# terraytherapeutics/COATI

Measured on AMD Instinct MI355X. Metric: molecules/sec (contrastive+AR train step), grande_closed, higher is better.
Workload: dtype bf16; 1 GPU; grande_closed d=256 L=16 nh=16 + E3GNN h=256x5, V=10322, batch 1024/GPU, seq_len 80, 16-atom point clouds, InfoNCE + AR loss, bf16 MFMA operands / fp32 accumulate + fp32 master weights, random-init weights; global_batch=1024, seq_len=80, parallelism=dp1

## Files before the change

### coati_amd/csrc/engine.cpp

```cpp
#include <stdarg.h>
#include <stdio.h>
#include <stdlib.h>
#include <string.h>

#include <algorithm>
#include <string>
#include <vector>

#include "../../include/coati_hip.h"
#include "kernels.h"

#define HIPCHK(x) do { hipError_t _h = (x); if (_h != hipSuccess) { coati_set_error("%s: %s", #x, hipGetErrorString(_h)); return COATI_EHIP; } } while (0)

static thread_local char g_err[512] = "";
void coati_set_error(const char* fmt, ...) {
  va_list ap;
  va_start(ap, fmt);
  vsnprintf(g_err, sizeof(g_err), fmt, ap);
  va_end(ap);
}
extern "C" const char* coati_last_error(void) { return g_err; }
extern "C" int coati_abi_version(void) { return COATI_ABI_VERSION; }

namespace {
// ... 1908 lines not shown
  COATI_CHECK_ARG(e->have_ws, "engine_infonce: needs the workspace of a forward / encode call");
  const size_t need = (size_t)2 * B * Bg;
  const size_t dh4_floats = (size_t)e->B * (e->T1 > e->T2 ? e->T1 : e->T2) * 4 * e->cfg.n_hidden_xformer * sizeof(bf16_t) / sizeof(float);
  COATI_CHECK_SHAPE(need <= e->nce_cap || need <= dh4_floats,
                    "engine_infonce: B=%d x Bg=%d does not fit the logits scratch (workspace was sized for Bg=%zu)", B, Bg,
                    e->nce_cap / (2 * (size_t)(e->B > 0 ? e->B : 1)));
  float* L1 = need <= e->nce_cap ? e->nce : reinterpret_cast<float*>(e->dh4);
  float* L2 = L1 + (size_t)B * Bg;
  COATI_TRY(launch_count_valid(bad_all, Bg, scal + 4, scal + 7, s));
  {
    SgemmBatch sb;
    COATI_TRY(sgemm_batch_add(sb, S_loc, E, 1, C_all, 1, E, L1, Bg, B, Bg, E, nullptr, 1.f, 0));
    COATI_TRY(sgemm_batch_add(sb, C_loc, E, 1, S_all, 1, E, L2, Bg, B, Bg, E, nullptr, 1.f, 0));
    COATI_TRY(launch_sgemm_batch(sb, s));
  }
  COATI_TRY(launch_infonce_rows2(L1, L2, Bg, B, Bg, row0, bad_all, scal + 2, scal + 3, scal + 7, gscale, s));
  {
    SgemmBatch sb;
    COATI_TRY(sgemm_batch_add(sb, L1, 1, Bg, S_loc, E, 1, dC_all, E, Bg, E, B, nullptr, 1.f, 0));
    COATI_TRY(sgemm_batch_add(sb, L2, 1, Bg, C_loc, E, 1, dS_all, E, Bg, E, B, nullptr, 1.f, 0));
    COATI_TRY(launch_sgemm_batch(sb, s));
  }
  {
    SgemmBatch sb;
    COATI_TRY(sgemm_batch_add(sb, L1, Bg, 1, C_all, E, 1, dS_all + (size_t)row0 * E, E, B, E, Bg, nullptr, 1.f, 1));
    COATI_TRY(sgemm_batch_add(sb, L2, Bg, 1, S_all, E, 1, dC_all + (size_t)row0 * E, E, B, E, Bg, nullptr, 1.f, 1));
    COATI_TRY(launch_sgemm_batch(sb, s));
  }
  return COATI_OK;
}

int coati_engine_backward(coati_engine* e, const float* dh_smiles, const float* dh_e3gnn, int stage, void* stream) {
  COATI_CHECK_ARG(e && !c2_refused(e), "engine_backward: a COATI2 engine bound without gradient and Adam buffers is inference-only (no backward)");
  COATI_CHECK_ARG(e->have_fwd && e->G, "engine_backward: no forward / gradient buffer");
  COATI_CHECK_ARG(stage >= 0 && stage <= 5, "engine_backward: bad stage");
  const bool c2 = e->enc_to_coati >= 0;
  COATI_CHECK_ARG(!c2 || dh_e3gnn == nullptr, "engine_backward: a COATI2 engine has no point encoder (dh_e3gnn must be null)");
  hipStream_t s = (hipStream_t)stream;
  const coati_config& c = e->cfg;
  const int C = c.n_hidden_xformer, H = c.n_hidden_e3nn, E = c.n_embd_common, B = e->B;
  if (stage == 0 || stage == 1) {
    const int M2 = e->p2.M;
    {
      GemmArgs a;
      memset(&a, 0, sizeof(a));
      a.A = e->p2.af; a.lda = C; a.B = e->S + e->lmhead; a.ldb = C; a.M = M2; a.N = c.n_tok; a.K = C;
      a.C = e->dlogits; a.ldc = e->Vpad; a.n_store = e->Vpad; a.lse = e->ce_lse; a.target = e->p2.packed ? e->p2.ypk : e->y_next; a.scal = e->scal;
      ProfScope ps(e, SITE_LMHEAD_DLOGITS, 2.0 * M2 * c.n_tok * C, s, (double)M2 * C * 2 + (double)c.n_tok * C * 2 + (double)M2 * e->Vpad * 2);
      COATI_TRY(gemm_rows(a, 0, EPI_CE_BWD, s));
    }
    COATI_TRY(wgrad(e, SITE_LMHEAD_WGRAD, e->dlogits, 0, e->Vpad, e->p2.af, C, M2, e->Vpad, C, e->G + e->lmhead, C, nullptr, c.n_tok, s));
    HIPCHK(hipMemsetAsync(e->dcliptok, 0, (size_t)B * E * sizeof(float), s));
    COATI_TRY(xformer_bwd(e, e->p2, e->da, 0, e->dcliptok, s, -1, 0, e->dlogits));
    if (dh_e3gnn) HIPCHK(hipMemcpyAsync(e->dhe, dh_e3gnn, (size_t)B * E * sizeof(float), hipMemcpyDeviceToDevice, s));
    else HIPCHK(hipMemsetAsync(e->dhe, 0, (size_t)B * E * sizeof(float), s));
    if (dh_smiles) HIPCHK(hipMemcpyAsync(e->dhs, dh_smiles, (size_t)B * E * sizeof(float), hipMemcpyDeviceToDevice, s));
    else HIPCHK(hipMemsetAsync(e->dhs, 0, (size_t)B * E * sizeof(float), s));
    if (c2) {
      COATI_TRY(launch_axpy(e->dcliptok, e->dhs, 1.f, (long long)B * E, s));
      COATI_TRY(coati2_head_bwd(e, e->c2t, e->c2t_sv, e->h_smiles, e->dcliptok, e->dhs, e->dhs, B, true, s));
      if (e->enc_to_coati > 0)
        COATI_TRY(coati2_head_bwd(e, e->c2s, e->c2s_sv, e->hstop, e->dhs, e->c2s.residual ? e->dhs : nullptr, e->dhstop, B, true, s));
    } else if (c.token_mlp) {
      HIPCHK(hipMemsetAsync(e->dptok, 0, (size_t)B * E * sizeof(float), s));
      HIPCHK(hipMemsetAsync(e->dstok, 0, (size_t)B * E * sizeof(float), s));
      COATI_TRY(launch_select_rows_bwd(e->use_point, e->dcliptok, e->dptok, e->dstok, B, E, s));
      SgemmBatch sb;
      COATI_TRY(head_linear_bwd(e, sb, e->dptok, e->sa, e->tokw, e->tokb, e->dsa, B, E, E));
      COATI_TRY(head_linear_bwd(e, sb, e->dstok, e->sb, e->tokw, e->tokb, e->dsb, B, E, E));
      COATI_TRY(launch_sgemm_batch(sb, s));
      COATI_TRY(launch_silu_bwd(e->h_e3gnn, e->dsa, e->dhe, (long long)B * E, 1, s));
      COATI_TRY(launch_silu_bwd(e->h_smiles, e->dsb, e->dhs, (long long)B * E, 1, s));
    } else {
      COATI_TRY(launch_select_rows_bwd(e->use_point, e->dcliptok, e->dhe, e->dhs, B, E, s));
    }
    const bool old_arch = c.norm_clips && c.old_architecture;
    if (e->enc_to_coati <= 0) {
    if (old_arch) {
      COATI_TRY(launch_layernorm_bwd(e->dhs, 1, E, e->hs_ln, E, 0, e->hs_mean, e->hs_rstd, e->P + e->s2c_lnw, nullptr, e->dhs_ln, nullptr, e->G + e->s2c_lnw, e->G + e->s2c_lnb, e->ln_partial, B, E, s));
      if (c.use_point_encoder)
        COATI_TRY(launch_layernorm_bwd(e->dhe, 1, E, e->hp_ln, E, 0, e->hp_mean, e->hp_rstd, e->P + e->p2c_lnw, nullptr, e->dhp_ln, nullptr, e->G + e->p2c_lnw, e->G + e->p2c_lnb, e->ln_partial, B, E, s));
    }
    {
      SgemmBatch sb;
      if (old_arch) COATI_TRY(head_linear_bwd(e, sb, e->dhs_ln, e->hstop, e->s2c_w, e->s2c_b, e->dhstop, B, E, C));
      else if (c.norm_clips) COATI_TRY(head_linear_bwd(e, sb, e->dhs, e->hs_ln, e->s2c_w, e->s2c_b, e->dhs_ln, B, E, C));
      else COATI_TRY(head_linear_bwd(e, sb, e->dhs, e->hstop, e->s2c_w, e->s2c_b, e->dhstop, B, E, C));
      if (c.use_point_encoder) {
        if (old_arch) COATI_TRY(head_linear_bwd(e, sb, e->dhp_ln, e->hpoint, e->p2c_w, e->p2c_b, e->dhpoint, B, E, H));
        else if (c.norm_clips) COATI_TRY(head_linear_bwd(e, sb, e->dhe, e->hp_ln, e->p2c_w, e->p2c_b, e->dhp_ln, B, E, H));
        else COATI_TRY(head_linear_bwd(e, sb, e->dhe, e->hpoint, e->p2c_w, e->p2c_b, e->dhpoint, B, E, H));
      }
      COATI_TRY(launch_sgemm_batch(sb, s));
    }
    if (c.norm_clips && !old_arch) {
      COATI_TRY(launch_layernorm_bwd(e->dhs_ln, 1, C, e->hstop, C, 0, e->hs_mean, e->hs_rstd, e->P + e->s2c_lnw, nullptr, e->dhstop, nullptr, e->G + e->s2c_lnw, e->G + e->s2c_lnb, e->ln_partial, B, C, s));
      if (c.use_point_encoder)
        COATI_TRY(launch_layernorm_bwd(e->dhp_ln, 1, H, e->hpoint, H, 0, e->hp_mean, e->hp_rstd, e->P + e->p2c_lnw, nullptr, e->dhpoint, nullptr, e->G + e->p2c_lnw, e->G + e->p2c_lnb, e->ln_partial, B, H, s));
    }
    }
  }
  const int Lx = c.n_layer_xformer, Lmid = Lx / 2;
  const bool ovl_bwd = (stage == 0 || stage == 2 || stage == 4) && (e->prof_mask == 0 || e->prof_keep_overlap) && c.use_point_encoder;
  if (stage == 0 || stage == 1) { e->gnn_bwd_done = false; e->gnn_side_pending = false; }
  if (ovl_bwd) {
    COATI_TRY(fork_side(e, s));
    COATI_TRY(gnn_bwd(e, e->dhpoint, e->side));
  }
  if (stage == 0 || stage == 2 || stage == 4) {
    if (e->p1.tail) {
      COATI_TRY(xformer_bwd(e, e->p1, e->dhstop, 1, nullptr, s, Lx, stage == 4 ? Lmid : 0));
    } else {
      float* dxf = reinterpret_cast<float*>(e->dh4);
      HIPCHK(hipMemsetAsync(dxf, 0, (size_t)e->p1.M * C * sizeof(float), s));
      COATI_TRY(launch_scatter_rows_add(e->dhstop, e->stop_pos, dxf, B, e->T1, C, s, e->p1.packed ? e->p1.off : nullptr));
      COATI_TRY(xformer_bwd(e, e->p1, dxf, 1, nullptr, s, Lx, stage == 4 ? Lmid : 0));
    }
  }
  if (stage == 5) COATI_TRY(xformer_bwd(e, e->p1, nullptr, 1, nullptr, s, Lmid, 0));
  if (ovl_bwd && stage == 4) {
    e->gnn_side_pending = true;
  } else if (ovl_bwd || (stage == 5 && e->gnn_side_pending)) {
    COATI_TRY(join_side(e, s));
    e->gnn_bwd_done = true;
    e->gnn_side_pending = false;
// ... 352 lines not shown
```

### coati_amd/csrc/gnn.hip

```cpp
#include "kernels.h"

#define IN_EPS 1e-5f

__global__ __launch_bounds__(256) void gnn_embed_kernel(const long long* __restrict__ atoms, const int* __restrict__ lut_ix,
                                                        const int* __restrict__ lut_iy, const float* __restrict__ W,
                                                        const float* __restrict__ bias, float* __restrict__ h32,
                                                        bf16_t* __restrict__ h16, long long ld16, float* __restrict__ rstd_out,
                                                        float* __restrict__ mask, int BA, int H, int* __restrict__ err) {
  const int lane = threadIdx.x & 63, wave = threadIdx.x >> 6;
  const int row = blockIdx.x * 4 + wave;
  if (row >= BA) return;
  long long z = atoms[row];
  if (lane == 0) mask[row] = z > 0 ? 1.f : 0.f;
  if (lut_ix == nullptr && z > 83 && lane == 0 && err != nullptr) atomicOr(err, 4);
  if (z < 0) z = 0;
  if (z > 119) z = 119;
  const bool table = lut_ix == nullptr;
  if (table && z > 83) z = 83;
  const int ix = table ? 0 : lut_ix[z], iy = table ? 0 : lut_iy[z];
  float e[16];
  float s = 0.f;
#pragma unroll
  for (int i = 0; i < 16; ++i) {
    const int c = lane + 64 * i;
    float v = 0.f;
    if (c < H) {
      if (table) {
        v = W[z * H + c];
      } else {
        v = bias[c];
        if (ix >= 0) v += W[c * 28 + ix];
        if (iy >= 0) v += W[c * 28 + iy];
      }
    }
    e[i] = v;
    s += v;
  }
  const float mean = wave_sum(s) / (float)H;
  float q = 0.f;
#pragma unroll
  for (int i = 0; i < 16; ++i)
    if (lane + 64 * i < H) q += (e[i] - mean) * (e[i] - mean);
  const float rstd = 1.0f / sqrtf(wave_sum(q) / (float)H + IN_EPS);
  if (lane == 0) rstd_out[row] = rstd;
#pragma unroll
  for (int i = 0; i < 16; ++i) {
    const int c = lane + 64 * i;
    if (c < H) {
      const float v = (e[i] - mean) * rstd;
      h32[(long long)row * H + c] = v;
      h16[(long long)row * ld16 + c] = f2bf(v);
    }
  }
}

int launch_gnn_embed(const long long* atoms, const int* lut_ix, const int* lut_iy, const float* W, const float* b,
                     float* h32, bf16_t* h16, long long ld16, float* rstd, float* mask, int BA, int H,
                     hipStream_t s, int* err) {
  COATI_CHECK_ARG(atoms && W && h32 && h16 && rstd && mask && ((lut_ix && lut_iy && b) || (!lut_ix && !lut_iy && !b)), "gnn_embed: null operand");
  COATI_CHECK_SHAPE(BA > 0 && H > 0 && H <= 1024, "gnn_embed: unsupported shape");
  hipLaunchKernelGGL(gnn_embed_kernel, dim3(cdiv(BA, 4)), dim3(256), 0, s, atoms, lut_ix, lut_iy, W, b, h32, h16, ld16, rstd, mask, BA, H, err);
  COATI_LAUNCH_CHECK("gnn_embed");
  return COATI_OK;
}

__global__ __launch_bounds__(256) void gnn_embed_bwd_kernel(const long long* __restrict__ atoms, const int* __restrict__ lut_ix,
                                                            const int* __restrict__ lut_iy, const float* __restrict__ de,
                                                            float* __restrict__ dW, float* __restrict__ db, int BA, int H,
                                                            int rows_per_chunk) {
  extern __shared__ float acc[];
  for (int i = threadIdx.x; i < 29 * H; i += blockDim.x) acc[i] = 0.f;
  __syncthreads();
  const int r0 = blockIdx.x * rows_per_chunk;
  int r1 = r0 + rows_per_chunk;
  if (r1 > BA) r1 = BA;
  for (int c = threadIdx.x; c < H; c += blockDim.x) {
    float bsum = 0.f;
    for (int row = r0; row < r1; ++row) {
      long long z = atoms[row];
      if (z < 0) z = 0;
      if (z > 119) z = 119;
      const int ix = lut_ix[z], iy = lut_iy[z];
      const float v = de[(long long)row * H + c];
      bsum += v;
      acc[ix * H + c] += v;
      if (iy != ix) acc[iy * H + c] += v;
    }
    acc[28 * H + c] = bsum;
  }
  __syncthreads();
  for (int f = threadIdx.x; f < 28 * H; f += blockDim.x) {
    const int c = f / 28, i = f - c * 28;
    const float v = acc[i * H + c];
    if (v != 0.f) atomicAdd(dW + f, v);
  }
  for (int c = threadIdx.x; c < H; c += blockDim.x) atomicAdd(db + c, acc[28 * H + c]);
}

__global__ __launch_bounds__(256) void gnn_embed_table_bwd_kernel(const long long* __restrict__ atoms, const float* __restrict__ de,
                                                                  float* __restrict__ dT, int BA, int H, int rows_per_chunk) {
  const int r0 = blockIdx.x * rows_per_chunk;
  int r1 = r0 + rows_per_chunk;
  if (r1 > BA) r1 = BA;
  for (int c = threadIdx.x; c < H; c += blockDim.x) {
    float run = 0.f;
    long long zr = -1;
    for (int row = r0; row < r1; ++row) {
      long long z = atoms[row];
      if (z < 0) z = 0;
      if (z > 83) z = 83;
      if (z != zr) {
        if (zr >= 0 && run != 0.f) atomicAdd(dT + zr * H + c, run);
        zr = z;
        run = 0.f;
      }
      run += de[(long long)row * H + c];
    }
    if (zr >= 0 && run != 0.f) atomicAdd(dT + zr * H + c, run);
  }
}

int launch_gnn_embed_bwd(const long long* atoms, const int* lut_ix, const int* lut_iy, const float* de,
                         float* dW, float* db, int BA, int H, hipStream_t s) {
  if (lut_ix == nullptr && lut_iy == nullptr && db == nullptr) {
    COATI_CHECK_ARG(atoms && de && dW, "gnn_embed_bwd: null operand");
    const int rpc = 32;
    hipLaunchKernelGGL(gnn_embed_table_bwd_kernel, dim3(cdiv(BA, rpc)), dim3(256), 0, s, atoms, de, dW, BA, H, rpc);
    COATI_LAUNCH_CHECK("gnn_embed_table_bwd");
    return COATI_OK;
  }
  COATI_CHECK_ARG(atoms && lut_ix && lut_iy && de && dW && db, "gnn_embed_bwd: null operand");
  COATI_CHECK_SHAPE((size_t)29 * H * 4 <= 64 * 1024, "gnn_embed_bwd: H=%d too wide for the LDS accumulator", H);
  const int chunks = BA >= 4096 ? 128 : (BA >= 256 ? 8 : 1);
  const int rpc = cdiv(BA, chunks);
  hipLaunchKernelGGL(gnn_embed_bwd_kernel, dim3(cdiv(BA, rpc)), dim3(256), (size_t)29 * H * 4, s, atoms, lut_ix, lut_iy, de, dW, db, BA, H, rpc);
  COATI_LAUNCH_CHECK("gnn_embed_bwd");
  return COATI_OK;
}

__global__ __launch_bounds__(256) void gnn_node_res_silu_kernel(const float* __restrict__ u32, const long long* __restrict__ atoms,
                                                                const int* __restrict__ lut_ix, const int* __restrict__ lut_iy,
                                                                const float* __restrict__ W3c, long long ldw, bf16_t* __restrict__ upre,
                                                                bf16_t* __restrict__ t16, int BA, int H) {
  const int row = blockIdx.x;
  if (row >= BA) return;
  long long z = atoms[row];
  if (z < 0) z = 0;
  if (z > 119) z = 119;
  const int ix = lut_ix[z], iy = lut_iy[z];
  for (int c = threadIdx.x; c < H; c += blockDim.x) {
    float v = u32[(long long)row * H + c];
    if (ix >= 0) v += W3c[c * ldw + ix];
    if (iy >= 0 && iy != ix) v += W3c[c * ldw + iy];
    upre[(long long)row * H + c] = f2bf(v);
    t16[(long long)row * H + c] = f2bf(silu_f(v));
  }
}

int launch_gnn_node_res_silu(const float* u32, const long long* atoms, const int* lut_ix, const int* lut_iy, const float* W3c, long long ldw,
                             bf16_t* upre, bf16_t* t16, int BA, int H, hipStream_t s) {
  COATI_CHECK_ARG(u32 && atoms && lut_ix && lut_iy && W3c && upre && t16, "gnn_node_res_silu: null operand");
  hipLaunchKernelGGL(gnn_node_res_silu_kernel, dim3(BA), dim3(256), 0, s, u32, atoms, lut_ix, lut_iy, W3c, ldw, upre, t16, BA, H);
  COATI_LAUNCH_CHECK("gnn_node_res_silu");
  return COATI_OK;
}

__global__ __launch_bounds__(256) void gnn_onehot_wgrad_kernel(const long long* __restrict__ atoms, const int* __restrict__ lut_ix,
                                                               const int* __restrict__ lut_iy, const bf16_t* __restrict__ du,
                                                               float* __restrict__ dW, long long ldw, int BA, int H, int rows_per_chunk) {
  extern __shared__ float acc[];
  for (int i = threadIdx.x; i < 28 * H; i += blockDim.x) acc[i] = 0.f;
// ... 385 lines not shown
```

### coati_amd/csrc/kernels.h

```cpp
#pragma once
#include "common.h"

enum CoatiEpi {
  EPI_BF16 = 0,
  EPI_F32 = 1,
  EPI_RES_F32 = 2,
  EPI_GELU = 3,
  EPI_DGELU = 4,
  EPI_SILU = 5,
  EPI_DSILU = 6,
  EPI_ACC_F32 = 7,
  EPI_CE_PARTIAL = 8,
  EPI_CE_BWD = 9,
  EPI_EDGE_DPRE = 10,
  EPI_QKV_ROPE = 11,
  EPI_GELU_GRAD = 12,
  EPI_MUL_AUX = 13,
  EPI_LNBWD = 14,
  EPI_CE_BWD_ROW = 15,
  EPI_CE_LSE = 16,
  EPI_COUNT = 17
};

struct GemmArgs {
// ... 224 lines not shown
int launch_topk_sample_prompt(const float* logits, long long ldl, int B, int V, int k, float inv_temp, const float* u,
                              const long long* prompt, long long ldp, const int* plen, int pos, long long* tok_out, int* stopped,
                              int stop_token, int pad_token, hipStream_t s);
int launch_topk_sample_rows(const float* logits, long long ldl, int B, int V, int k, float inv_temp, const float* u, long long ldu,
                            const long long* prompt, long long ldp, const int* plen, const int* req, int* pos, long long* out,
                            long long ldo, long long* tok_next, int* done, int Tmax, int stop_token, hipStream_t s);
int launch_kv_cache_fill_rows(const bf16_t* qkv, bf16_t* cache, const int* row_src, int R, int B, int T, int n_head, int head_size,
                              int Tmax, hipStream_t s);
int launch_gather_last_rows(const float* x, const int* off, float* out, int B, int C, int R, hipStream_t s);
int launch_kv_cache_fill(const bf16_t* qkv, bf16_t* cache, int B, int m, int n_head, int head_size, int Tmax, hipStream_t s);
int launch_batch_ncols(const long long* tok, int B, int S, int* ncols, hipStream_t s);
int launch_batch_tail(const long long* tok, int B, int S, int ncol, long long* tok_out, long long* y_out,
                      const long long* masked, int n_masked, hipStream_t s);

int launch_ce_finish(const float2* partial, int tiles_n, const bf16_t* a, long long lda, const bf16_t* W,
                     long long ldw, const long long* target, float* lse, float* scal, int M, int C, int V,
                     hipStream_t s);
int launch_ce_lse_finish(const bf16_t* a, long long lda, const bf16_t* W, long long ldw, const long long* target, const float* lse,
                         float* scal, int M, int C, int V, hipStream_t s);
int launch_ce_lse_finish_picked(const long long* target, const float* lse, const float* tl, float* scal, int M, int V, hipStream_t s);
int launch_ce_seq(const float2* partial, int tiles_n, const bf16_t* a, long long lda, const bf16_t* W, long long ldw,
                  const long long* target, const int* off, float* nll, int B, int T, int C, int V, hipStream_t s);
int launch_ce_seq_bwd(const float2* partial, int tiles_n, const bf16_t* a, long long lda, const bf16_t* W, long long ldw,
                      const long long* target, const int* off, const float* weights, float* nll, float* lse, float* row_scale, int B, int T,
                      int C, int V, hipStream_t s);

int launch_gnn_embed(const long long* atoms, const int* lut_ix, const int* lut_iy, const float* W, const float* b,
                     float* h32, bf16_t* h16, long long ld16, float* rstd, float* mask, int BA, int H,
                     hipStream_t s, int* err = nullptr);
int launch_gnn_node_res_silu(const float* u32, const long long* atoms, const int* lut_ix, const int* lut_iy, const float* W3c, long long ldw,
                             bf16_t* upre, bf16_t* t16, int BA, int H, hipStream_t s);
int launch_gnn_onehot_wgrad(const long long* atoms, const int* lut_ix, const int* lut_iy, const bf16_t* du, float* dW, long long ldw, int BA,
                            int H, hipStream_t s);
int launch_gnn_embed_bwd(const long long* atoms, const int* lut_ix, const int* lut_iy, const float* de,
                         float* dW, float* db, int BA, int H, hipStream_t s);
int launch_gnn_geom(const float* coords, const float* mask, float cutoff, float* d2, float* w, int B, int A,
                    hipStream_t s);
int launch_gnn_compact(const float* w_dense, const float* d2_dense, int* seg, int* n_edges, int* e_bj, int* e_bk, int* e_rev,
                       float* e_d2, float* e_w, int* pos, int B, int A, hipStream_t s);
int launch_gnn_edge_pre_c(const bf16_t* P, long long ldp, const int* seg, const int* e_bk, const float* e_d2, const float* w1c,
                          long long w1c_stride, const float* b1, bf16_t* e1, int BA, int H, hipStream_t s);
int launch_gnn_edge_reduce_c(const bf16_t* s2, const int* seg, const float* e_w, bf16_t* mi, long long ldmi, int BA, int H, hipStream_t s);
int launch_gnn_edge_fwd_fused(const bf16_t* P, long long ldp, const int* seg, const int* e_bk, const float* e_d2, const float* e_w,
                              const float* w1c, long long w1c_stride, const float* b1, const bf16_t* W3, long long ldw, const float* b3,
                              bf16_t* e1, bf16_t* s2, bf16_t* mi, long long ldmi, int BA, int H, hipStream_t s);
int launch_gnn_edge_reduce_bwd_c(const bf16_t* dmi, long long lddmi, const bf16_t* s2, const int* seg, const float* e_w,
                                 bf16_t* ds2, int BA, int H, hipStream_t s);
int launch_gnn_edge_pre_bwd_c(const bf16_t* dpre, const int* seg, const int* e_rev, const float* e_d2, bf16_t* dP, long long lddp,
                              float* dw1c, long long dw1c_stride, float* db1, int BA, int H, hipStream_t s);
int launch_gnn_readout(const float* o, const float* mask, float* hp, int B, int A, int H, hipStream_t s);
int launch_gnn_readout_bwd(const float* dhp, const float* mask, bf16_t* dout, int B, int A, int H, hipStream_t s);

int launch_silu_fwd(const float* x, float* y, long long n, hipStream_t s);
int launch_silu_bwd(const float* x, const float* dy, float* dx, long long n, int accumulate, hipStream_t s);
int launch_swiglu(const float* u, long long ldu, float* g, long long ldg, int B, int N, hipStream_t s);
int launch_swiglu_bwd(const float* u, long long ldu, const float* dg, long long lddg, float* du, long long lddu, int B, int N, hipStream_t s);
int launch_group_mean_rows(const float* x, long long ldx, const int* off, const float* w, const float* fallback, float* out, int G, int E,
                           hipStream_t s);
int launch_select_rows(const unsigned char* use_a, const float* a, const float* b, float* out, int B, int C,
                       hipStream_t s);
int launch_select_rows_bwd(const unsigned char* use_a, const float* dout, float* da, float* db, int B, int C,
                           hipStream_t s);
int launch_axpy(const float* x, float* y, float alpha, long long n, hipStream_t s);
int launch_infonce_rows2(float* logits, float* logits2, long long ld, int R, int N, int label0, const unsigned char* bad,
                         float* loss_sum, float* loss_sum2, const float* inv_count, float gscale, hipStream_t s);
int launch_infonce_rows(float* logits, long long ld, int R, int N, int label0, const unsigned char* bad,
                        float* loss_sum, const float* inv_count, float gscale, hipStream_t s);
int launch_count_valid(const unsigned char* bad, int n, float* out_count, float* out_inv, hipStream_t s);
int launch_colsum2(const float* a, const float* b2, const unsigned char* bad, float* out, int B, int E, hipStream_t s);
int launch_center_rows(const float* z, const unsigned char* bad, const float* sum, const float* count, float* zc, int B, int E, hipStream_t s);
int launch_standardize(const float* z, const unsigned char* bad, const float* stats, const float* count, float* zt, float* rsigma,
                       int B, int E, hipStream_t s);
int launch_barlow_dc(float* C, const float* count, float lam, float* loss, int E, hipStream_t s);
int launch_standardize_bwd(const float* dzt, const float* zt, const unsigned char* bad, const float* rsigma, const float* m,
                           const float* count, float scale, float* dz, int B, int E, hipStream_t s);

int launch_grad_sqnorm(const float* g, long long n, float* partial, int n_partial, float* out_norm, float max_norm,
                       float* out_coef, hipStream_t s);
int launch_adamw(float* p, const float* g, float* m, float* v, bf16_t* shadow, long long n, float lr, float b1,
                 float b2, float eps, float wd, int step, const float* coef, float gscale, hipStream_t s, const int* skip = nullptr);
int launch_cast_bf16(const float* src, bf16_t* dst, long long n, hipStream_t s);
int launch_transpose_cast(const float* src, long long ld_src, bf16_t* dst, long long ld_dst, int rows, int cols,
                          hipStream_t s);
int launch_pack_rows_cast(const float* src, long long ld_src, bf16_t* dst, long long ld_dst, int rows, int cols,
                          hipStream_t s);

struct ShadowJob {
  long long src_off, dst_off;
  int ld_src, ld_dst, rows, cols, transpose;
};
int launch_shadow_jobs(const ShadowJob* jobs, const int* tile_start, int n_jobs, int n_tiles, const float* P, bf16_t* S,
                       hipStream_t s);
```

### coati_amd/csrc/loss.hip

```cpp
#include "kernels.h"

__global__ void silu_fwd_kernel(const float* __restrict__ x, float* __restrict__ y, long long n) {
  const long long i = (long long)blockIdx.x * blockDim.x + threadIdx.x;
  if (i < n) y[i] = silu_f(x[i]);
}
int launch_silu_fwd(const float* x, float* y, long long n, hipStream_t s) {
  COATI_CHECK_ARG(x && y, "silu_fwd: null operand");
  hipLaunchKernelGGL(silu_fwd_kernel, dim3(cdiv(n, 256)), dim3(256), 0, s, x, y, n);
  COATI_LAUNCH_CHECK("silu_fwd");
  return COATI_OK;
}

template <bool V4>
__global__ __launch_bounds__(256) void swiglu_kernel(const float* __restrict__ u, long long ldu, float* __restrict__ g, long long ldg,
                                                     int B, int N) {
  const int W = V4 ? N / 4 : N;
  const long long i = (long long)blockIdx.x * blockDim.x + threadIdx.x;
  if (i >= (long long)B * W) return;
  const long long b = i / W;
  const int j = (int)(i - b * W);
  const float* r = u + b * ldu;
  if constexpr (V4) {
    const float4 x = *reinterpret_cast<const float4*>(r + 4 * j);
    const float4 q = *reinterpret_cast<const float4*>(r + N + 4 * j);
// ... 35 lines not shown
    float4 dx, dq;
    swiglu_bwd_f(x.x, q.x, d.x, dx.x, dq.x);
    swiglu_bwd_f(x.y, q.y, d.y, dx.y, dq.y);
    swiglu_bwd_f(x.z, q.z, d.z, dx.z, dq.z);
    swiglu_bwd_f(x.w, q.w, d.w, dx.w, dq.w);
    *reinterpret_cast<float4*>(o + 4 * j) = dx;
    *reinterpret_cast<float4*>(o + N + 4 * j) = dq;
  } else {
    swiglu_bwd_f(r[j], r[N + j], dg[b * lddg + j], o[j], o[N + j]);
  }
}
int launch_swiglu_bwd(const float* u, long long ldu, const float* dg, long long lddg, float* du, long long lddu, int B, int N, hipStream_t s) {
  COATI_CHECK_ARG(u && dg && du, "swiglu_bwd: null operand");
  COATI_CHECK_SHAPE(B > 0 && N > 0 && ldu >= 2LL * N && lddg >= N && lddu >= 2LL * N, "swiglu_bwd: bad shape B=%d N=%d ldu=%lld lddg=%lld lddu=%lld", B, N,
                    ldu, lddg, lddu);
  const bool v4 = N % 4 == 0 && ldu % 4 == 0 && lddg % 4 == 0 && lddu % 4 == 0 && reinterpret_cast<uintptr_t>(u) % 16 == 0 &&
                  reinterpret_cast<uintptr_t>(dg) % 16 == 0 && reinterpret_cast<uintptr_t>(du) % 16 == 0;
  const long long n = (long long)B * (v4 ? N / 4 : N);
  if (v4) hipLaunchKernelGGL(swiglu_bwd_kernel<true>, dim3(cdiv(n, 256)), dim3(256), 0, s, u, ldu, dg, lddg, du, lddu, B, N);
  else hipLaunchKernelGGL(swiglu_bwd_kernel<false>, dim3(cdiv(n, 256)), dim3(256), 0, s, u, ldu, dg, lddg, du, lddu, B, N);
  COATI_LAUNCH_CHECK("swiglu_bwd");
  return COATI_OK;
}

__global__ __launch_bounds__(256) void group_mean_rows_kernel(const float* __restrict__ x, long long ldx, const int* __restrict__ off,
                                                              const float* __restrict__ w, const float* __restrict__ fallback,
                                                              float* __restrict__ out, int E) {
  const int g = blockIdx.x;
  const int lo = off[g], hi = off[g + 1];
  float* o = out + (long long)g * E;
  if (hi <= lo) {
    for (int e = threadIdx.x; e < E; e += blockDim.x) o[e] = fallback[(long long)g * E + e];
    return;
  }
  float ws = 0.f;
  for (int i = lo; i < hi; ++i) ws += w ? w[i] : 1.f;
  const float inv = 1.f / ws;
  for (int e = threadIdx.x; e < E; e += blockDim.x) {
    float acc = 0.f;
    for (int i = lo; i < hi; ++i) acc += (w ? w[i] : 1.f) * x[(long long)i * ldx + e];
    o[e] = acc * inv;
  }
}
int launch_group_mean_rows(const float* x, long long ldx, const int* off, const float* w, const float* fallback, float* out, int G, int E,
                           hipStream_t s) {
  COATI_CHECK_ARG(x && off && fallback && out, "group_mean_rows: null operand");
  COATI_CHECK_SHAPE(G > 0 && E > 0 && ldx >= E, "group_mean_rows: bad shape G=%d E=%d ldx=%lld", G, E, ldx);
  hipLaunchKernelGGL(group_mean_rows_kernel, dim3(G), dim3(E < 256 ? (E + 63) / 64 * 64 : 256), 0, s, x, ldx, off, w, fallback, out, E);
  COATI_LAUNCH_CHECK("group_mean_rows");
  return COATI_OK;
}

__global__ void silu_bwd_kernel(const float* __restrict__ x, const float* __restrict__ dy, float* __restrict__ dx,
                                long long n, int accumulate) {
  const long long i = (long long)blockIdx.x * blockDim.x + threadIdx.x;
  if (i < n) {
    const float g = dy[i] * dsilu_f(x[i]);
    dx[i] = accumulate ? dx[i] + g : g;
  }
}
int launch_silu_bwd(const float* x, const float* dy, float* dx, long long n, int accumulate, hipStream_t s) {
  COATI_CHECK_ARG(x && dy && dx, "silu_bwd: null operand");
  hipLaunchKernelGGL(silu_bwd_kernel, dim3(cdiv(n, 256)), dim3(256), 0, s, x, dy, dx, n, accumulate);
  COATI_LAUNCH_CHECK("silu_bwd");
  return COATI_OK;
}

__global__ void select_rows_kernel(const unsigned char* __restrict__ use_a, const float* __restrict__ a,
                                   const float* __restrict__ b, float* __restrict__ out, int B, int C) {
  const long long i = (long long)blockIdx.x * blockDim.x + threadIdx.x;
  if (i < (long long)B * C) out[i] = use_a[i / C] ? a[i] : b[i];
}
int launch_select_rows(const unsigned char* use_a, const float* a, const float* b, float* out, int B, int C, hipStream_t s) {
  COATI_CHECK_ARG(use_a && a && b && out, "select_rows: null operand");
  hipLaunchKernelGGL(select_rows_kernel, dim3(cdiv((long long)B * C, 256)), dim3(256), 0, s, use_a, a, b, out, B, C);
  COATI_LAUNCH_CHECK("select_rows");
  return COATI_OK;
}

__global__ void select_rows_bwd_kernel(const unsigned char* __restrict__ use_a, const float* __restrict__ dout,
                                       float* __restrict__ da, float* __restrict__ db, int B, int C) {
  const long long i = (long long)blockIdx.x * blockDim.x + threadIdx.x;
  if (i < (long long)B * C) {
    if (use_a[i / C]) da[i] += dout[i]; else db[i] += dout[i];
  }
}
int launch_select_rows_bwd(const unsigned char* use_a, const float* dout, float* da, float* db, int B, int C, hipStream_t s) {
  COATI_CHECK_ARG(use_a && dout && da && db, "select_rows_bwd: null operand");
  hipLaunchKernelGGL(select_rows_bwd_kernel, dim3(cdiv((long long)B * C, 256)), dim3(256), 0, s, use_a, dout, da, db, B, C);
  COATI_LAUNCH_CHECK("select_rows_bwd");
  return COATI_OK;
}

__global__ void axpy_kernel(const float* __restrict__ x, float* __restrict__ y, float alpha, long long n) {
  const long long i = (long long)blockIdx.x * blockDim.x + threadIdx.x;
  if (i < n) y[i] += alpha * x[i];
}
int launch_axpy(const float* x, float* y, float alpha, long long n, hipStream_t s) {
  COATI_CHECK_ARG(x && y, "axpy: null operand");
  hipLaunchKernelGGL(axpy_kernel, dim3(cdiv(n, 256)), dim3(256), 0, s, x, y, alpha, n);
  COATI_LAUNCH_CHECK("axpy");
  return COATI_OK;
}

template <int NR>
__global__ __launch_bounds__(256) void infonce_rows_kernel(float* __restrict__ logits, float* __restrict__ logits2, long long ld, int R, int N,
                                                           int label0, const unsigned char* __restrict__ bad, float* __restrict__ loss_sum,
                                                           float* __restrict__ loss_sum2, const float* __restrict__ inv_count, float gscale) {
  const int lane = threadIdx.x & 63, r = blockIdx.x * 4 + (threadIdx.x >> 6);
  if (r >= R) return;
  float* row = (blockIdx.y ? logits2 : logits) + (long long)r * ld;
  float* ls = blockIdx.y ? loss_sum2 : loss_sum;
  const int label = label0 + r;
  if (bad[label]) {
    for (int c = lane; c < N; c += 64) row[c] = 0.f;
    return;
  }
  const float g = gscale * inv_count[0];
  if constexpr (NR > 0) {
    float v[NR];
#pragma unroll
    for (int i = 0; i < NR; ++i) v[i] = lane + 64 * i < N ? row[lane + 64 * i] : -INFINITY;
    float mx = -INFINITY;
#pragma unroll
    for (int i = 0; i < NR; ++i) mx = fmaxf(mx, v[i]);
    mx = wave_max(mx);
    float sm = 0.f;
#pragma unroll
    for (int i = 0; i < NR; ++i) sm += __expf(v[i] - mx);
    sm = wave_sum(sm);
    const float lse = mx + __logf(sm);
    float at_label = 0.f;
#pragma unroll
    for (int i = 0; i < NR; ++i) {
      const int c = lane + 64 * i;
      float p = __expf(v[i] - lse);
      if (c == label) { at_label = v[i]; p -= 1.f; }
      if (c < N) row[c] = p * g;
    }
    at_label = wave_sum(at_label);
    if (lane == 0) atomicAdd(ls, lse - at_label);
  } else {
    float mx = -INFINITY;
    for (int c = lane; c < N; c += 64) mx = fmaxf(mx, row[c]);
    mx = wave_max(mx);
    float sm = 0.f;
    for (int c = lane; c < N; c += 64) sm += __expf(row[c] - mx);
    sm = wave_sum(sm);
    const float lse = mx + __logf(sm);
    if (lane == 0) atomicAdd(ls, lse - row[label]);
    __builtin_amdgcn_wave_barrier();
    for (int c = lane; c < N; c += 64) {
      float p = __expf(row[c] - lse);
      if (c == label) p -= 1.f;
      row[c] = p * g;
    }
  }
}
int launch_infonce_rows2(float* logits, float* logits2, long long ld, int R, int N, int label0, const unsigned char* bad,
                         float* loss_sum, float* loss_sum2, const float* inv_count, float gscale, hipStream_t s) {
  COATI_CHECK_ARG(logits && bad && loss_sum && inv_count && (logits2 == nullptr || loss_sum2 != nullptr), "infonce_rows: null operand");
  COATI_CHECK_SHAPE(R > 0 && N > 0 && label0 >= 0 && label0 + R <= N, "infonce_rows: labels out of range");
  const dim3 grid(cdiv(R, 4), logits2 ? 2 : 1);
  if (N <= 64 * 16) hipLaunchKernelGGL(infonce_rows_kernel<16>, grid, dim3(256), 0, s, logits, logits2, ld, R, N, label0, bad, loss_sum, loss_sum2, inv_count, gscale);
  else if (N <= 64 * 32) hipLaunchKernelGGL(infonce_rows_kernel<32>, grid, dim3(256), 0, s, logits, logits2, ld, R, N, label0, bad, loss_sum, loss_sum2, inv_count, gscale);
  else hipLaunchKernelGGL(infonce_rows_kernel<0>, grid, dim3(256), 0, s, logits, logits2, ld, R, N, label0, bad, loss_sum, loss_sum2, inv_count, gscale);
  COATI_LAUNCH_CHECK("infonce_rows");
  return COATI_OK;
}
int launch_infonce_rows(float* logits, long long ld, int R, int N, int label0, const unsigned char* bad,
                        float* loss_sum, const float* inv_count, float gscale, hipStream_t s) {
  return launch_infonce_rows2(logits, nullptr, ld, R, N, label0, bad, loss_sum, nullptr, inv_count, gscale, s);
}

__global__ void count_valid_kernel(const unsigned char* __restrict__ bad, int n, float* __restrict__ out_count,
                                   float* __restrict__ out_inv) {
  __shared__ int red[4];
  int c = 0;
  for (int i = threadIdx.x; i < n; i += blockDim.x) c += bad[i] ? 0 : 1;
  for (int o = 32; o > 0; o >>= 1) c += __shfl_xor(c, o, 64);
  if ((threadIdx.x & 63) == 0) red[threadIdx.x >> 6] = c;
  __syncthreads();
  if (threadIdx.x == 0) {
    const int t = red[0] + red[1] + red[2] + red[3];
    out_count[0] = (float)t;
    out_inv[0] = t > 0 ? 1.0f / (float)t : 0.f;
  }
}
int launch_count_valid(const unsigned char* bad, int n, float* out_count, float* out_inv, hipStream_t s) {
  COATI_CHECK_ARG(bad && out_count && out_inv, "count_valid: null operand");
  hipLaunchKernelGGL(count_valid_kernel, dim3(1), dim3(256), 0, s, bad, n, out_count, out_inv);
  COATI_LAUNCH_CHECK("count_valid");
  return COATI_OK;
}

__global__ __launch_bounds__(256) void colsum2_kernel(const float* __restrict__ a, const float* __restrict__ b2,
                                                      const unsigned char* __restrict__ bad, float* __restrict__ out, int B, int E) {
  __shared__ float red[2][4][64];
  const int c = blockIdx.x * 64 + (threadIdx.x & 63), rg = threadIdx.x >> 6;
  float s1 = 0.f, s2 = 0.f;
  if (c < E)
    for (int r = rg; r < B; r += 4) {
      if (bad[r]) continue;
      const float x = a[(long long)r * E + c];
      s1 += x;
      s2 += x * (b2 ? b2[(long long)r * E + c] : x);
    }
  red[0][rg][threadIdx.x & 63] = s1;
  red[1][rg][threadIdx.x & 63] = s2;
  __syncthreads();
  if (rg == 0 && c < E) {
    const int t = threadIdx.x;
    out[c] = red[0][0][t] + red[0][1][t] + red[0][2][t] + red[0][3][t];
    out[E + c] = red[1][0][t] + red[1][1][t] + red[1][2][t] + red[1][3][t];
  }
}
int launch_colsum2(const float* a, const float* b2, const unsigned char* bad, float* out, int B, int E, hipStream_t s) {
  COATI_CHECK_ARG(a && bad && out, "colsum2: null operand");
  hipLaunchKernelGGL(colsum2_kernel, dim3(cdiv(E, 64)), dim3(256), 0, s, a, b2, bad, out, B, E);
// ... 80 lines not shown
```

Baseline: 49870 molecules/s.

## Fuse grad-buffer init into select/silu bwd, batch atom loads, block-reduce InfoNCE loss

Several small backward-pass changes land together. The token_mlp head path drops four memset/memcpy calls: select_rows_bwd now writes fresh values, and silu_bwd writes base+grad directly. The GNN embedding backward kernels load atom indices once per 64-row tile, broadcast them with readlane, and batch eight gradient loads per step to cut serial dependent loads. InfoNCE moves to 8-wave blocks and reduces the loss in shared memory, so it issues one atomic per block instead of one per row.

```diff
diff --git a/coati_amd/csrc/engine.cpp b/coati_amd/csrc/engine.cpp
--- a/coati_amd/csrc/engine.cpp
+++ b/coati_amd/csrc/engine.cpp
@@ -1984,25 +1984,26 @@
     COATI_TRY(wgrad(e, SITE_LMHEAD_WGRAD, e->dlogits, 0, e->Vpad, e->p2.af, C, M2, e->Vpad, C, e->G + e->lmhead, C, nullptr, c.n_tok, s));
     HIPCHK(hipMemsetAsync(e->dcliptok, 0, (size_t)B * E * sizeof(float), s));
     COATI_TRY(xformer_bwd(e, e->p2, e->da, 0, e->dcliptok, s, -1, 0, e->dlogits));
-    if (dh_e3gnn) HIPCHK(hipMemcpyAsync(e->dhe, dh_e3gnn, (size_t)B * E * sizeof(float), hipMemcpyDeviceToDevice, s));
-    else HIPCHK(hipMemsetAsync(e->dhe, 0, (size_t)B * E * sizeof(float), s));
-    if (dh_smiles) HIPCHK(hipMemcpyAsync(e->dhs, dh_smiles, (size_t)B * E * sizeof(float), hipMemcpyDeviceToDevice, s));
-    else HIPCHK(hipMemsetAsync(e->dhs, 0, (size_t)B * E * sizeof(float), s));
+    const bool dh_fresh = !c2 && c.token_mlp;
+    if (!dh_fresh) {
+      if (dh_e3gnn) HIPCHK(hipMemcpyAsync(e->dhe, dh_e3gnn, (size_t)B * E * sizeof(float), hipMemcpyDeviceToDevice, s));
+      else HIPCHK(hipMemsetAsync(e->dhe, 0, (size_t)B * E * sizeof(float), s));
+      if (dh_smiles) HIPCHK(hipMemcpyAsync(e->dhs, dh_smiles, (size_t)B * E * sizeof(float), hipMemcpyDeviceToDevice, s));
+      else HIPCHK(hipMemsetAsync(e->dhs, 0, (size_t)B * E * sizeof(float), s));
+    }
     if (c2) {
       COATI_TRY(launch_axpy(e->dcliptok, e->dhs, 1.f, (long long)B * E, s));
       COATI_TRY(coati2_head_bwd(e, e->c2t, e->c2t_sv, e->h_smiles, e->dcliptok, e->dhs, e->dhs, B, true, s));
       if (e->enc_to_coati > 0)
         COATI_TRY(coati2_head_bwd(e, e->c2s, e->c2s_sv, e->hstop, e->dhs, e->c2s.residual ? e->dhs : nullptr, e->dhstop, B, true, s));
     } else if (c.token_mlp) {
-      HIPCHK(hipMemsetAsync(e->dptok, 0, (size_t)B * E * sizeof(float), s));
-      HIPCHK(hipMemsetAsync(e->dstok, 0, (size_t)B * E * sizeof(float), s));
-      COATI_TRY(launch_select_rows_bwd(e->use_point, e->dcliptok, e->dptok, e->dstok, B, E, s));
+      COATI_TRY(launch_select_rows_bwd(e->use_point, e->dcliptok, e->dptok, e->dstok, B, E, s, 1));
       SgemmBatch sb;
       COATI_TRY(head_linear_bwd(e, sb, e->dptok, e->sa, e->tokw, e->tokb, e->dsa, B, E, E));
       COATI_TRY(head_linear_bwd(e, sb, e->dstok, e->sb, e->tokw, e->tokb, e->dsb, B, E, E));
       COATI_TRY(launch_sgemm_batch(sb, s));
-      COATI_TRY(launch_silu_bwd(e->h_e3gnn, e->dsa, e->dhe, (long long)B * E, 1, s));
-      COATI_TRY(launch_silu_bwd(e->h_smiles, e->dsb, e->dhs, (long long)B * E, 1, s));
+      COATI_TRY(launch_silu_bwd(e->h_e3gnn, e->dsa, e->dhe, (long long)B * E, 2, s, dh_e3gnn));
+      COATI_TRY(launch_silu_bwd(e->h_smiles, e->dsb, e->dhs, (long long)B * E, 2, s, dh_smiles));
     } else {
       COATI_TRY(launch_select_rows_bwd(e->use_point, e->dcliptok, e->dhe, e->dhs, B, E, s));
     }
diff --git a/coati_amd/csrc/gnn.hip b/coati_amd/csrc/gnn.hip
--- a/coati_amd/csrc/gnn.hip
+++ b/coati_amd/csrc/gnn.hip
@@ -64,6 +64,7 @@
   return COATI_OK;
 }
 
+#define GNN_EB_DEPTH 8
 __global__ __launch_bounds__(256) void gnn_embed_bwd_kernel(const long long* __restrict__ atoms, const int* __restrict__ lut_ix,
                                                             const int* __restrict__ lut_iy, const float* __restrict__ de,
                                                             float* __restrict__ dW, float* __restrict__ db, int BA, int H,
@@ -71,22 +72,41 @@
   extern __shared__ float acc[];
   for (int i = threadIdx.x; i < 29 * H; i += blockDim.x) acc[i] = 0.f;
   __syncthreads();
+  const int lane = threadIdx.x & 63;
   const int r0 = blockIdx.x * rows_per_chunk;
   int r1 = r0 + rows_per_chunk;
   if (r1 > BA) r1 = BA;
-  for (int c = threadIdx.x; c < H; c += blockDim.x) {
+  for (int cb = 0; cb < H; cb += blockDim.x) {
+    const int c = cb + threadIdx.x;
+    const bool on = c < H;
     float bsum = 0.f;
-    for (int row = r0; row < r1; ++row) {
-      long long z = atoms[row];
-      if (z < 0) z = 0;
-      if (z > 119) z = 119;
-      const int ix = lut_ix[z], iy = lut_iy[z];
-      const float v = de[(long long)row * H + c];
-      bsum += v;
-      acc[ix * H + c] += v;
-      if (iy != ix) acc[iy * H + c] += v;
-    }
-    acc[28 * H + c] = bsum;
+    for (int rt = r0; rt < r1; rt += 64) {
+      int my_ix = -1, my_iy = -1;
+      if (rt + lane < r1) {
+        long long z = atoms[rt + lane];
+        if (z < 0) z = 0;
+        if (z > 119) z = 119;
+        my_ix = lut_ix[z];
+        my_iy = lut_iy[z];
+      }
+      const int n = r1 - rt < 64 ? r1 - rt : 64;
+      for (int j0 = 0; j0 < n; j0 += GNN_EB_DEPTH) {
+        float v[GNN_EB_DEPTH];
+#pragma unroll
+        for (int u = 0; u < GNN_EB_DEPTH; ++u) v[u] = (on && j0 + u < n) ? de[(long long)(rt + j0 + u) * H + c] : 0.f;
+#pragma unroll
+        for (int u = 0; u < GNN_EB_DEPTH; ++u) {
+          if (j0 + u >= n) break;
+          const int ix = __builtin_amdgcn_readlane(my_ix, j0 + u), iy = __builtin_amdgcn_readlane(my_iy, j0 + u);
+          if (on) {
+            bsum += v[u];
+            if (ix >= 0) acc[ix * H + c] += v[u];
+            if (iy >= 0 && iy != ix) acc[iy * H + c] += v[u];
+          }
+        }
+      }
+    }
+    if (on) acc[28 * H + c] = bsum;
   }
   __syncthreads();
   for (int f = threadIdx.x; f < 28 * H; f += blockDim.x) {
@@ -99,24 +119,42 @@
 
 __global__ __launch_bounds__(256) void gnn_embed_table_bwd_kernel(const long long* __restrict__ atoms, const float* __restrict__ de,
                                                                   float* __restrict__ dT, int BA, int H, int rows_per_chunk) {
+  const int lane = threadIdx.x & 63;
   const int r0 = blockIdx.x * rows_per_chunk;
   int r1 = r0 + rows_per_chunk;
   if (r1 > BA) r1 = BA;
-  for (int c = threadIdx.x; c < H; c += blockDim.x) {
+  for (int cb = 0; cb < H; cb += blockDim.x) {
+    const int c = cb + threadIdx.x;
+    const bool on = c < H;
     float run = 0.f;
-    long long zr = -1;
-    for (int row = r0; row < r1; ++row) {
-      long long z = atoms[row];
-      if (z < 0) z = 0;
-      if (z > 83) z = 83;
-      if (z != zr) {
-        if (zr >= 0 && run != 0.f) atomicAdd(dT + zr * H + c, run);
-        zr = z;
-        run = 0.f;
-      }
-      run += de[(long long)row * H + c];
-    }
-    if (zr >= 0 && run != 0.f) atomicAdd(dT + zr * H + c, run);
+    int zr = -1;
+    for (int rt = r0; rt < r1; rt += 64) {
+      int my_z = 0;
+      if (rt + lane < r1) {
+        long long z = atoms[rt + lane];
+        if (z < 0) z = 0;
+        if (z > 83) z = 83;
+        my_z = (int)z;
+      }
+      const int n = r1 - rt < 64 ? r1 - rt : 64;
+      for (int j0 = 0; j0 < n; j0 += GNN_EB_DEPTH) {
+        float v[GNN_EB_DEPTH];
+#pragma unroll
+        for (int u = 0; u < GNN_EB_DEPTH; ++u) v[u] = (on && j0 + u < n) ? de[(long long)(rt + j0 + u) * H + c] : 0.f;
+#pragma unroll
+        for (int u = 0; u < GNN_EB_DEPTH; ++u) {
+          if (j0 + u >= n) break;
+          const int z = __builtin_amdgcn_readlane(my_z, j0 + u);
+          if (z != zr) {
+            if (on && zr >= 0 && run != 0.f) atomicAdd(dT + (long long)zr * H + c, run);
+            zr = z;
+            run = 0.f;
+          }
+          run += v[u];
+        }
+      }
+    }
+    if (on && zr >= 0 && run != 0.f) atomicAdd(dT + (long long)zr * H + c, run);
   }
 }
 
diff --git a/coati_amd/csrc/kernels.h b/coati_amd/csrc/kernels.h
--- a/coati_amd/csrc/kernels.h
+++ b/coati_amd/csrc/kernels.h
@@ -300,7 +300,7 @@
 int launch_gnn_readout_bwd(const float* dhp, const float* mask, bf16_t* dout, int B, int A, int H, hipStream_t s);
 
 int launch_silu_fwd(const float* x, float* y, long long n, hipStream_t s);
-int launch_silu_bwd(const float* x, const float* dy, float* dx, long long n, int accumulate, hipStream_t s);
+int launch_silu_bwd(const float* x, const float* dy, float* dx, long long n, int accumulate, hipStream_t s, const float* base = nullptr);
 int launch_swiglu(const float* u, long long ldu, float* g, long long ldg, int B, int N, hipStream_t s);
 int launch_swiglu_bwd(const float* u, long long ldu, const float* dg, long long lddg, float* du, long long lddu, int B, int N, hipStream_t s);
 int launch_group_mean_rows(const float* x, long long ldx, const int* off, const float* w, const float* fallback, float* out, int G, int E,
@@ -308,7 +308,7 @@
 int launch_select_rows(const unsigned char* use_a, const float* a, const float* b, float* out, int B, int C,
                        hipStream_t s);
 int launch_select_rows_bwd(const unsigned char* use_a, const float* dout, float* da, float* db, int B, int C,
-                           hipStream_t s);
+                           hipStream_t s, int fresh = 0);
 int launch_axpy(const float* x, float* y, float alpha, long long n, hipStream_t s);
 int launch_infonce_rows2(float* logits, float* logits2, long long ld, int R, int N, int label0, const unsigned char* bad,
                          float* loss_sum, float* loss_sum2, const float* inv_count, float gscale, hipStream_t s);
diff --git a/coati_amd/csrc/loss.hip b/coati_amd/csrc/loss.hip
--- a/coati_amd/csrc/loss.hip
+++ b/coati_amd/csrc/loss.hip
@@ -111,16 +111,17 @@
 }
 
 __global__ void silu_bwd_kernel(const float* __restrict__ x, const float* __restrict__ dy, float* __restrict__ dx,
-                                long long n, int accumulate) {
+                                long long n, int accumulate, const float* __restrict__ base) {
   const long long i = (long long)blockIdx.x * blockDim.x + threadIdx.x;
   if (i < n) {
     const float g = dy[i] * dsilu_f(x[i]);
-    dx[i] = accumulate ? dx[i] + g : g;
-  }
-}
-int launch_silu_bwd(const float* x, const float* dy, float* dx, long long n, int accumulate, hipStream_t s) {
-  COATI_CHECK_ARG(x && dy && dx, "silu_bwd: null operand");
-  hipLaunchKernelGGL(silu_bwd_kernel, dim3(cdiv(n, 256)), dim3(256), 0, s, x, dy, dx, n, accumulate);
+    if (accumulate == 2) dx[i] = (base ? base[i] : 0.f) + g;
+    else dx[i] = accumulate ? dx[i] + g : g;
+  }
+}
+int launch_silu_bwd(const float* x, const float* dy, float* dx, long long n, int accumulate, hipStream_t s, const float* base) {
+  COATI_CHECK_ARG(x && dy && dx && accumulate >= 0 && accumulate <= 2 && (accumulate == 2 || !base), "silu_bwd: null operand / bad mode");
+  hipLaunchKernelGGL(silu_bwd_kernel, dim3(cdiv(n, 256)), dim3(256), 0, s, x, dy, dx, n, accumulate, base);
   COATI_LAUNCH_CHECK("silu_bwd");
   return COATI_OK;
 }
@@ -138,15 +139,24 @@
 }
 
 __global__ void select_rows_bwd_kernel(const unsigned char* __restrict__ use_a, const float* __restrict__ dout,
-                                       float* __restrict__ da, float* __restrict__ db, int B, int C) {
+                                       float* __restrict__ da, float* __restrict__ db, int B, int C, int fresh) {
   const long long i = (long long)blockIdx.x * blockDim.x + threadIdx.x;
   if (i < (long long)B * C) {
-    if (use_a[i / C]) da[i] += dout[i]; else db[i] += dout[i];
-  }
-}
-int launch_select_rows_bwd(const unsigned char* use_a, const float* dout, float* da, float* db, int B, int C, hipStream_t s) {
+    const bool a = use_a[i / C] != 0;
+    if (fresh) {
+      const float v = 0.f + dout[i];
+      da[i] = a ? v : 0.f;
+      db[i] = a ? 0.f : v;
+    } else if (a) {
+      da[i] += dout[i];
+    } else {
+      db[i] += dout[i];
+    }
+  }
+}
+int launch_select_rows_bwd(const unsigned char* use_a, const float* dout, float* da, float* db, int B, int C, hipStream_t s, int fresh) {
   COATI_CHECK_ARG(use_a && dout && da && db, "select_rows_bwd: null operand");
-  hipLaunchKernelGGL(select_rows_bwd_kernel, dim3(cdiv((long long)B * C, 256)), dim3(256), 0, s, use_a, dout, da, db, B, C);
+  hipLaunchKernelGGL(select_rows_bwd_kernel, dim3(cdiv((long long)B * C, 256)), dim3(256), 0, s, use_a, dout, da, db, B, C, fresh);
   COATI_LAUNCH_CHECK("select_rows_bwd");
   return COATI_OK;
 }
@@ -162,68 +172,79 @@
   return COATI_OK;
 }
 
+#define NCE_WAVES 8
 template <int NR>
-__global__ __launch_bounds__(256) void infonce_rows_kernel(float* __restrict__ logits, float* __restrict__ logits2, long long ld, int R, int N,
+__global__ __launch_bounds__(64 * NCE_WAVES) void infonce_rows_kernel(float* __restrict__ logits, float* __restrict__ logits2, long long ld, int R, int N,
                                                            int label0, const unsigned char* __restrict__ bad, float* __restrict__ loss_sum,
                                                            float* __restrict__ loss_sum2, const float* __restrict__ inv_count, float gscale) {
-  const int lane = threadIdx.x & 63, r = blockIdx.x * 4 + (threadIdx.x >> 6);
-  if (r >= R) return;
-  float* row = (blockIdx.y ? logits2 : logits) + (long long)r * ld;
-  float* ls = blockIdx.y ? loss_sum2 : loss_sum;
-  const int label = label0 + r;
-  if (bad[label]) {
-    for (int c = lane; c < N; c += 64) row[c] = 0.f;
-    return;
-  }
-  const float g = gscale * inv_count[0];
-  if constexpr (NR > 0) {
-    float v[NR];
-#pragma unroll
-    for (int i = 0; i < NR; ++i) v[i] = lane + 64 * i < N ? row[lane + 64 * i] : -INFINITY;
-    float mx = -INFINITY;
-#pragma unroll
-    for (int i = 0; i < NR; ++i) mx = fmaxf(mx, v[i]);
-    mx = wave_max(mx);
-    float sm = 0.f;
-#pragma unroll
-    for (int i = 0; i < NR; ++i) sm += __expf(v[i] - mx);
-    sm = wave_sum(sm);
-    const float lse = mx + __logf(sm);
-    float at_label = 0.f;
-#pragma unroll
-    for (int i = 0; i < NR; ++i) {
-      const int c = lane + 64 * i;
-      float p = __expf(v[i] - lse);
-      if (c == label) { at_label = v[i]; p -= 1.f; }
-      if (c < N) row[c] = p * g;
+  __shared__ float red[NCE_WAVES];
+  const int lane = threadIdx.x & 63, wave = threadIdx.x >> 6, r = blockIdx.x * NCE_WAVES + wave;
+  float term = 0.f;
+  if (r < R) {
+    float* row = (blockIdx.y ? logits2 : logits) + (long long)r * ld;
+    const int label = label0 + r;
+    if (bad[label]) {
+      for (int c = lane; c < N; c += 64) row[c] = 0.f;
+    } else {
+      const float g = gscale * inv_count[0];
+      if constexpr (NR > 0) {
+        float v[NR];
+#pragma unroll
+        for (int i = 0; i < NR; ++i) v[i] = lane + 64 * i < N ? row[lane + 64 * i] : -INFINITY;
+        float mx = -INFINITY;
+#pragma unroll
+        for (int i = 0; i < NR; ++i) mx = fmaxf(mx, v[i]);
+        mx = wave_max(mx);
+        float sm = 0.f;
+#pragma unroll
+        for (int i = 0; i < NR; ++i) sm += __expf(v[i] - mx);
+        sm = wave_sum(sm);
+        const float lse = mx + __logf(sm);
+        float at_label = 0.f;
+#pragma unroll
+        for (int i = 0; i < NR; ++i) {
+          const int c = lane + 64 * i;
+          float p = __expf(v[i] - lse);
+          if (c == label) { at_label = v[i]; p -= 1.f; }
+          if (c < N) row[c] = p * g;
+        }
+        at_label = wave_sum(at_label);
+        term = lse - at_label;
+      } else {
+        float mx = -INFINITY;
+        for (int c = lane; c < N; c += 64) mx = fmaxf(mx, row[c]);
+        mx = wave_max(mx);
+        float sm = 0.f;
+        for (int c = lane; c < N; c += 64) sm += __expf(row[c] - mx);
+        sm = wave_sum(sm);
+        const float lse = mx + __logf(sm);
+        term = lse - row[label];
+        __builtin_amdgcn_wave_barrier();
+        for (int c = lane; c < N; c += 64) {
+          float p = __expf(row[c] - lse);
+          if (c == label) p -= 1.f;
+          row[c] = p * g;
+        }
+      }
     }
-    at_label = wave_sum(at_label);
-    if (lane == 0) atomicAdd(ls, lse - at_label);
-  } else {
-    float mx = -INFINITY;
-    for (int c = lane; c < N; c += 64) mx = fmaxf(mx, row[c]);
-    mx = wave_max(mx);
-    float sm = 0.f;
-    for (int c = lane; c < N; c += 64) sm += __expf(row[c] - mx);
-    sm = wave_sum(sm);
-    const float lse = mx + __logf(sm);
-    if (lane == 0) atomicAdd(ls, lse - row[label]);
-    __builtin_amdgcn_wave_barrier();
-    for (int c = lane; c < N; c += 64) {
-      float p = __expf(row[c] - lse);
-      if (c == label) p -= 1.f;
-      row[c] = p * g;
-    }
+  }
+  if (lane == 0) red[wave] = term;
+  __syncthreads();
+  if (threadIdx.x == 0) {
+    float sum = 0.f;
+#pragma unroll
+    for (int w = 0; w < NCE_WAVES; ++w) sum += red[w];
+    atomicAdd(blockIdx.y ? loss_sum2 : loss_sum, sum);
   }
 }
 int launch_infonce_rows2(float* logits, float* logits2, long long ld, int R, int N, int label0, const unsigned char* bad,
                          float* loss_sum, float* loss_sum2, const float* inv_count, float gscale, hipStream_t s) {
   COATI_CHECK_ARG(logits && bad && loss_sum && inv_count && (logits2 == nullptr || loss_sum2 != nullptr), "infonce_rows: null operand");
   COATI_CHECK_SHAPE(R > 0 && N > 0 && label0 >= 0 && label0 + R <= N, "infonce_rows: labels out of range");
-  const dim3 grid(cdiv(R, 4), logits2 ? 2 : 1);
-  if (N <= 64 * 16) hipLaunchKernelGGL(infonce_rows_kernel<16>, grid, dim3(256), 0, s, logits, logits2, ld, R, N, label0, bad, loss_sum, loss_sum2, inv_count, gscale);
-  else if (N <= 64 * 32) hipLaunchKernelGGL(infonce_rows_kernel<32>, grid, dim3(256), 0, s, logits, logits2, ld, R, N, label0, bad, loss_sum, loss_sum2, inv_count, gscale);
-  else hipLaunchKernelGGL(infonce_rows_kernel<0>, grid, dim3(256), 0, s, logits, logits2, ld, R, N, label0, bad, loss_sum, loss_sum2, inv_count, gscale);
+  const dim3 grid(cdiv(R, NCE_WAVES), logits2 ? 2 : 1);
+  if (N <= 64 * 16) hipLaunchKernelGGL(infonce_rows_kernel<16>, grid, dim3(64 * NCE_WAVES), 0, s, logits, logits2, ld, R, N, label0, bad, loss_sum, loss_sum2, inv_count, gscale);
+  else if (N <= 64 * 32) hipLaunchKernelGGL(infonce_rows_kernel<32>, grid, dim3(64 * NCE_WAVES), 0, s, logits, logits2, ld, R, N, label0, bad, loss_sum, loss_sum2, inv_count, gscale);
+  else hipLaunchKernelGGL(infonce_rows_kernel<0>, grid, dim3(64 * NCE_WAVES), 0, s, logits, logits2, ld, R, N, label0, bad, loss_sum, loss_sum2, inv_count, gscale);
   COATI_LAUNCH_CHECK("infonce_rows");
   return COATI_OK;
 }
```

Measured after the change: 49890 molecules/s, median of 2. No clear change (+0.0%).
